# phirling/pyc2ray

Hardware: AMD Instinct MI355X
Metric: cell-updates/sec (raytrace+chem) (higher is better)
Workload: dtype f64

## Files before the change

### pyc2ray_amd/csrc/api.hip

```cpp
#include "asora_internal.hpp"

#include <chrono>

namespace asora {

static State g_state;
static std::string g_error;

State &state() { return g_state; }
int fail(int code, const std::string &msg) { g_error = msg; return code; }
void clear_error() { g_error.clear(); }

static int flush_timers()
{
    State &st = g_state;
    if (st.pending_timers.empty()) return 0;
    ASORA_HIP_TRY(hipStreamSynchronize(st.stream));
    for (hipStream_t s : st.side) if (s) ASORA_HIP_TRY(hipStreamSynchronize(s));
    for (auto &pt : st.pending_timers) {
        float ms = 0.f;
        if (hipEventElapsedTime(&ms, pt.e0, pt.e1) == hipSuccess) {
            st.k_ms[pt.which] += (double)ms;
            st.k_n[pt.which] += 1;
        }
// ... 63 lines not shown
    st.th_on = false; st.th = ThermalConsts();
    drop(st.grid[ASORA_GRID_CLUMP]);
    st.clump_mode = 0; st.clump_c = 1.0;
    st.lls_a = st.lls_b = 0.0;
    st.plane = PlaneFluxSet{};
    drop(st.budget_partial);
    if (st.budget_host) { (void)hipHostFree(st.budget_host); st.budget_host = nullptr; }
    drop(st.bubble_mask); drop(st.bubble_rows); drop(st.bubble_scan); drop(st.bubble_partial); drop(st.bubble_result); drop(st.bubble_edges);
    if (st.bubble_host) { (void)hipHostFree(st.bubble_host); st.bubble_host = nullptr; }
    drop(st.region_label); drop(st.region_volume); drop(st.region_flags); drop(st.region_result);
    drop(st.topo_complement);
    for (int g = 0; g < ASORA_GRID_COUNT; ++g) { st.grid[g] = nullptr; st.grid_valid[g] = false; }
    st.nhi = st.staging = st.acc = nullptr;
    drop(st.arena); st.arena_bytes = 0;
    st.ev_clean[0] = st.ev_clean[1] = false; st.ev_sets_known = false;
    drop(st.reach.mask); drop(st.reach.count_dev); st.reach = State::ReachMask();
    st.ev_open = false;
    st.temp_probe_valid = false;
    st.nhi_t = st.phi_t = st.heat_t = nullptr;
    st.have_heat_tables = false;
    drop(st.tables); st.table_len = 0; st.num_spec = 1; st.spec_stride = 0;
    drop(st.src_spec); drop(st.src_spec_sorted); st.src_spec_max = 0;
    drop(st.src_pos); drop(st.src_flux); drop(st.src_pos_sorted); drop(st.src_flux_sorted); st.src_i0_sorted.clear(); st.num_src = 0;
    st.src_pos_host.clear(); st.src_pos_sorted_host.clear();
    release_pair_lists(st);
    drop(st.shell_scratch); st.shell_scratch_bytes = 0;
    drop(st.sb_trail); st.sb_trail_bytes = 0;
    if (st.geom_patch_dev) { (void)hipFree(st.geom_patch_dev); st.geom_patch_dev = nullptr; st.geom_patch_cap = 0; }
    drop(st.sb_active); drop(st.sb_nbox); drop(st.sb_loss); drop(st.sb_loss_final); st.subbox_cap = 0;
    release_geometry(st);
// ... 23 lines not shown

int check_planes(const char *who, int code, const char *tail, int i_begin, int i_count)
{
    if (i_begin < 0 || i_count < 0 || i_begin + i_count > g_state.N) return fail(code, std::string(who) + ": " + tail);
    return 0;
}

int check_sources(const char *who, int code, const std::string &tail, int src_begin, int src_count)
{
    if (src_begin < 0 || src_count < 0 || src_begin + src_count > g_state.num_src) return fail(code, std::string(who) + ": " + tail);
    return 0;
}

int require_grids(const char *who, std::initializer_list<int> grids)
{
    for (int g : grids)
        if (!g_state.grid_valid[g]) return fail(4, std::string(who) + ": grid " + std::to_string(g) + " holds no data");
    return 0;
}

}

using namespace asora;

extern "C" {

constexpr int ARENA_CANDIDATES = 8;
constexpr int ARENA_SLOTS = 14;
__global__ void __launch_bounds__(256) placement_probe_kernel(char *arena, size_t slot, size_t n)
{
    const double *in[5]; double *out[7];
    for (int q = 0; q < 5; ++q) in[q] = reinterpret_cast<const double *>(arena + q * slot);
// ... 183 lines not shown
```

### pyc2ray_amd/csrc/asora_internal.hpp

```cpp
#pragma once
#include <hip/hip_runtime.h>
#include <algorithm>
#include <cmath>
#include <cstdint>
#include <cstdio>
#include <cstdlib>
#include <cstring>
#include <initializer_list>
#include <string>
#include <vector>

#include "../../include/asora_hip.h"
#include "raytrace_plan.hpp"

namespace asora {

struct OctGeomDev {
    const uint4 *cellA;
    const uint4 *cellB;
    int nsteps;
    int info;
    int inner;
    int reserved_;
};
// ... 183 lines not shown
    unsigned long long *topo_complement = nullptr;

    unsigned long long *counters = nullptr;
    long long last_gamma_cells = 0, last_eval_cells = 0;

    double *acc = nullptr;
    char *arena = nullptr;
    size_t arena_bytes = 0;
    int arena_candidates = 0;
    double arena_probe_ms = 0.0, arena_probe_worst_ms = 0.0;
    double arena_probe_wall_ms = 0.0, device_init_wall_ms = 0.0;
    int ev_base = 0;
    bool ev_clean[2] = {false, false};
    bool ev_sets_known = false;
    int ev_folded_iter = -1;
    EvolveStatus *ev_status = nullptr;
    EvolveStatus *ev_host = nullptr;
    bool ev_open = false, ev_first = true;
    double *temp_probe_dev = nullptr;
    double temp_probe[5] = {0, 0, 0, 0, 0};
    bool temp_probe_valid = false;
    double temp_consts[4] = {0, 0, 0, 0};
    int ev_reported = 0;
    int ev_enqueued = 0;
    double ev_chem[6] = {0, 0, 0, 0, 0, 0};
    int ev_src_begin = 0, ev_src_count = 0;
    RtParams ev_rt;
    bool ev_slab = false;
    int ev_own_begin = 0, ev_own_count = 0;
    bool ev_slab_passed = false;
// ... 190 lines not shown
int launch_fold_out(State &st, const double *a, const double *a_t, double *out, double *z_a, double *z_t, int i_begin, int i_count,
                    const int *done);
int launch_fold_out_pair(State &st, const double *a, const double *a_t, double *out, double *z_a, double *z_t, const double *h,
                         const double *h_t, double *hout, double *zh_a, double *zh_t, int i_begin, int i_count, const int *done);
int launch_add_planes(State &st, double *dst, const double *src, size_t n, const int *done);
int launch_convergence_test(State &st, const double *sums, EvolveStatus *status);
int launch_reach_mask(State &st, const int32_t *src_pos, int src_begin, int src_count, double R, unsigned char *mask, size_t bytes_one_layout);
int launch_reach_count(State &st, const unsigned char *mask, size_t bytes_both_layouts, unsigned long long *out_dev);

int ensure_runtime();
int require_init(const char *who);
int check_N(const char *who, int N);
int check_planes(const char *who, int code, const char *tail, int i_begin, int i_count);
int check_sources(const char *who, int code, const std::string &tail, int src_begin, int src_count);
int require_grids(const char *who, std::initializer_list<int> grids);
int ensure_optional_grid(int which);
int reset_counters();
int require_raytrace_inputs(const char *who, double R, int NumTau, bool density, bool xh_av);
void fill_rt_params(RtParams &p, double R, double sig, double dr, double minlogtau, double dlogtau, int NumTau, int radius_path = 0);
inline void use_source_list(RtParams &p, const State &st, bool sorted)
{
    p.src_pos = sorted ? st.src_pos_sorted : st.src_pos;
    p.src_flux = sorted ? st.src_flux_sorted : st.src_flux;
    p.src_spec = sorted ? st.src_spec_sorted : st.src_spec;
}
int check_source_spectra(const char *who);
void sort_sources_by_position(const int32_t *pos, int NumSrc, std::vector<int> &order);
int ensure_red_capacity(size_t entries);
int ensure_temp_probe(double bh00, double albpow, double colh0, double temph0);
ChemTileParams chem_tile_common(int i_begin, int i_count, const double chem[6]);
// ... 9 lines not shown
```

### pyc2ray_amd/csrc/bubble_mfp.hip

```cpp
#include "asora_internal.hpp"

#pragma clang fp contract(off)

namespace asora {

constexpr int BM_THREADS = 256;
constexpr int BM_WAVES = BM_THREADS / 64;
constexpr int BM_SCAN_THREADS = 1024;
constexpr int BM_SLOTS = ASORA_BUBBLE_MAX_BINS + 5;
constexpr int BM_UNDER = ASORA_BUBBLE_MAX_BINS, BM_OVER = BM_UNDER + 1, BM_ENDED = BM_UNDER + 2, BM_CAPPED = BM_UNDER + 3,
              BM_LEFT = BM_UNDER + 4;
constexpr int BM_RESULT = BM_SLOTS + 3;
constexpr int BM_BLOCKS_PER_CU = 8;
static_assert(BM_RESULT + ASORA_BUBBLE_MAX_BINS + 1 <= BUBBLE_HOST_WORDS, "the pinned area holds the result words and the edges");

__global__ void __launch_bounds__(BM_THREADS) bubble_mask_kernel(const double *__restrict__ x, int N, int W, double threshold, int phase,
                                                                 unsigned long long *__restrict__ mask, unsigned *__restrict__ rows)
{
    const int lane = threadIdx.x & 63;
    const size_t nrows = (size_t)N * N, nwaves = (size_t)gridDim.x * BM_WAVES;
    for (size_t row = (size_t)blockIdx.x * BM_WAVES + (threadIdx.x >> 6); row < nrows; row += nwaves) {
        const double *q = x + row * (size_t)N;
        unsigned long long mine = 0;
        unsigned count = 0;
// ... 225 lines not shown
        ASORA_HIP_TRY(hipGetLastError());
    }
    if (!scan) return 0;
    KernelTimer kt(ASORA_KERNEL_BUBBLE_SCAN);
    hipLaunchKernelGGL(bubble_scan_kernel, dim3(1), dim3(BM_SCAN_THREADS), 0, st.stream, (const unsigned *)st.bubble_rows, nrows,
                       st.bubble_scan);
    ASORA_HIP_TRY(hipGetLastError());
    return 0;
}

int check_bubble_grid(const char *who, int which, double threshold, int phase)
{
    const State &st = state();
    if (which < 0 || which >= ASORA_GRID_COUNT) return fail(3, std::string(who) + ": bad grid selector");
    if (!st.grid[which] || !st.grid_valid[which]) return fail(4, std::string(who) + ": grid " + std::to_string(which) + " holds no data");
    if (!std::isfinite(threshold)) return fail(3, std::string(who) + ": the threshold must be finite");
    if (phase != 0 && phase != 1) return fail(3, std::string(who) + ": phase must be 0 (x >= threshold) or 1 (x < threshold)");
    return 0;
}

struct BubbleRecord {
    int32_t *start = nullptr, *status = nullptr;
    double *dir = nullptr, *len = nullptr;
    ~BubbleRecord() { (void)hipFree(start); (void)hipFree(status); (void)hipFree(dir); (void)hipFree(len); }
};

}

using namespace asora;

// ... 96 lines not shown
```

### pyc2ray_amd/csrc/chemistry_api.hip

```cpp
#include "asora_internal.hpp"

namespace asora {

int ensure_temp_probe(double bh00, double albpow, double colh0, double temph0)
{
    State &st = state();
    const double clump = st.clump_mode == 1 ? st.clump_c : 1.0;
    const double b = clump * bh00;
    const double c[4] = {b, albpow, colh0, temph0};
    if (st.temp_probe_valid && std::memcmp(c, st.temp_consts, sizeof c) == 0 && st.temp_probe_clump == clump) return 0;
    if (!st.temp_probe_dev) ASORA_HIP_TRY(hipMalloc(&st.temp_probe_dev, sizeof(double) * 8));
    if (int rc = launch_temp_probe(st, st.grid[ASORA_GRID_TEMP], st.ncell, b, albpow, colh0, temph0, st.temp_probe_dev)) return rc;
    ASORA_HIP_TRY(hipMemcpyAsync(st.temp_probe, st.temp_probe_dev, sizeof(double) * 5, hipMemcpyDeviceToHost, st.stream));
    ASORA_HIP_TRY(hipStreamSynchronize(st.stream));
    std::memcpy(st.temp_consts, c, sizeof c);
    st.temp_probe_clump = clump;
    st.temp_probe_valid = true;
    return 0;
}

ChemTileParams chem_tile_common(int i_begin, int i_count, const double chem[6])
{
    State &st = state();
    ChemTileParams p;
// ... 35 lines not shown

using namespace asora;

extern "C" {

int asora_chemistry_device(double dt, double bh00, double albpow, double colh0, double temph0, double abu_c,
                           int *conv_flag, double *sum_xh1, double *sum_xh0)
{
    clear_error();
    if (int rc = require_init("chemistry_device")) return rc;
    State &st = state();
    if (int rc = require_grids("chemistry_device", {ASORA_GRID_NDENS, ASORA_GRID_TEMP, ASORA_GRID_XH, ASORA_GRID_XH_AV, ASORA_GRID_PHI_ION})) return rc;
    if (st.th_on) {
        if (!st.grid[ASORA_GRID_PHI_HEAT] || !st.grid_valid[ASORA_GRID_PHI_HEAT])
            return fail(4, "chemistry_device: thermal mode needs the heating rates (ASORA_GRID_PHI_HEAT) on the device");
        if (int rc = ensure_optional_grid(ASORA_GRID_TEMP_END)) return rc;
    }
    st.grid_valid[ASORA_GRID_XH_INTERMED] = true;
    ChemParams p;
    p.ncell = st.ncell;
    p.dt = dt; p.bh00 = bh00; p.albpow = albpow; p.colh0 = colh0; p.temph0 = temph0; p.abu_c = abu_c;
    p.ndens = st.grid[ASORA_GRID_NDENS]; p.temp = st.grid[ASORA_GRID_TEMP]; p.xh = st.grid[ASORA_GRID_XH];
    p.phi = st.grid[ASORA_GRID_PHI_ION];
    p.xh_av = st.grid[ASORA_GRID_XH_AV]; p.xh_intermed = st.grid[ASORA_GRID_XH_INTERMED];
    p.red_partial = st.red_partial; p.red_final = st.red_final; p.red_blocks = st.red_blocks;
    if (st.th_on) {
        p.thermal = true; p.th = st.th;
        p.phi_heat = st.grid[ASORA_GRID_PHI_HEAT]; p.temp_end = st.grid[ASORA_GRID_TEMP_END]; p.th_stats = st.th_stats_dev;
        ASORA_HIP_TRY(hipMemsetAsync(st.th_stats_dev, 0, 3 * sizeof(unsigned long long), st.stream));
        st.grid_valid[ASORA_GRID_TEMP_END] = true;
// ... 158 lines not shown
```

### pyc2ray_amd/csrc/evolve_api.hip

```cpp
#include "asora_internal.hpp"

namespace asora {

static double *acc_pair(int set) { return state().acc + (size_t)set * 2 * state().ncell; }
static double *heat_pair(int set) { return state().heat_acc + (size_t)set * 2 * state().ncell; }

static int ensure_heat_acc()
{
    State &st = state();
    if (st.heat_acc) return 0;
    ASORA_HIP_TRY(hipMalloc(&st.heat_acc, 4 * st.ncell * sizeof(double)));
    ASORA_HIP_TRY(hipMemsetAsync(st.heat_acc, 0, 4 * st.ncell * sizeof(double), st.stream));
    st.heat_clean[0] = st.heat_clean[1] = true;
    return 0;
}

static int ensure_heat_outbox()
{
    State &st = state();
    if (st.heat_outbox) return 0;
    ASORA_HIP_TRY(hipMalloc(&st.heat_outbox, st.ncell * sizeof(double)));
    return 0;
}

// ... 102 lines not shown
    if (st.th_on) {
        if (!st.have_heat_tables || st.opt[ASORA_OPT_GREY_NOTABLES])
            return fail(4, "evolve_begin: thermal mode needs heating tables on the device (heat_table_to_device)");
        if (!st.opt[ASORA_OPT_Z_TRANSPOSED]) return fail(4, "evolve_begin: thermal mode needs the [k][j][i] twins (ASORA_OPT_Z_TRANSPOSED = 1)");
        if (int rc = ensure_optional_grid(ASORA_GRID_PHI_HEAT)) return rc;
        if (int rc = ensure_optional_grid(ASORA_GRID_TEMP_END)) return rc;
        if (int rc = ensure_heat_acc()) return rc;
        if (slab) { if (int rc = ensure_heat_outbox()) return rc; }
    }
    if (int rc = check_plane_flux(st, st.plane, "evolve_begin", false, st.th_on)) return rc;
    if (slab && st.plane.count > 0 && !(own_begin == 0 && own_count == st.N))
        return fail(4, "evolve_begin_slab: a plane-parallel flux (asora_plane_flux) needs a step that owns every plane (the full-grid "
                       "exchange, asora_evolve_slab_fold_all): the slab exchange does not deliver a whole-box sweep");
    if (int rc = ensure_temp_probe(bh00, albpow, colh0, temph0)) return rc;

    if (!st.ev_sets_known || slab)
        if (int rc = zero_pairs_unless_clean()) return rc;
    if (slab) st.reach.in_use = false;
    else if (int rc = decide_reach_mask(src_begin, src_count, R, st.plane.count > 0)) return rc;

    if (!st.ev_clean[0] && !st.ev_clean[1]) return fail(11, "evolve_begin: no clean accumulator pair (internal error)");
    st.ev_base = st.ev_clean[0] ? 0 : 1;
    if (st.th_on) {
        if (int rc = zero_pairs_unless_clean(true)) return rc;
        ASORA_HIP_TRY(hipMemsetAsync(st.th_stats_dev, 0, 3 * sizeof(unsigned long long), st.stream));
    }
    st.ev_folded_iter = 0;
    if (!st.ev_status) {
        ASORA_HIP_TRY(hipMalloc(&st.ev_status, sizeof(EvolveStatus)));
        ASORA_HIP_TRY(hipHostMalloc(&st.ev_host, sizeof(EvolveStatus), hipHostMallocDefault));
// ... 97 lines not shown
    if (st.ev_slab_thermal) {
        p.heat = slab_heat_pair(0);
        st.heat_clean[0] = st.heat_clean[1] = false;
    }
    return launch_raytrace(st, p, false, st.ev_slab_thermal);
}

int asora_evolve_slab_fold_out(int i_begin, int i_count)
{
    clear_error();
    if (int rc = require_slab("evolve_slab_fold_out")) return rc;
    State &st = state();
    if (int rc = check_planes("evolve_slab_fold_out", 4, "bad plane range", i_begin, i_count)) return rc;
    if (i_count > 0 && i_begin < st.ev_own_begin + st.ev_own_count && st.ev_own_begin < i_begin + i_count)
        return fail(4, "evolve_slab_fold_out: the range holds planes this rank owns (their rates stay: the pass folds them)");
    st.ev_sets_known = false;
    double *cur = slab_pair(0), *nxt = slab_pair(1);
    if (st.ev_slab_thermal) {
        double *hcur = slab_heat_pair(0), *hnxt = slab_heat_pair(1);
        return launch_fold_out_pair(st, cur, cur + st.ncell, st.staging, nxt, nxt + st.ncell, hcur, hcur + st.ncell, st.heat_outbox,
                                    hnxt, hnxt + st.ncell, i_begin, i_count, &st.ev_status->done);
    }
    return launch_fold_out(st, cur, cur + st.ncell, st.staging, nxt, nxt + st.ncell, i_begin, i_count, &st.ev_status->done);
}

int asora_evolve_slab_fold_all(void)
{
    clear_error();
    if (int rc = require_slab("evolve_slab_fold_all")) return rc;
    State &st = state();
    if (st.ev_slab_passed) return fail(4, "evolve_slab_fold_all: the iteration's pass has been enqueued already");
    if (st.ev_own_begin != 0 || st.ev_own_count != st.N)
        return fail(4, "evolve_slab_fold_all: the step must own every plane (asora_evolve_begin_slab(..., 0, N)): the chemistry is replicated");
    st.ev_sets_known = false;
    st.ev_rates_in_outbox = true; st.ev_folded_all = true;
    double *cur = slab_pair(0), *nxt = slab_pair(1);
    if (st.ev_slab_thermal) {
        double *hcur = slab_heat_pair(0), *hnxt = slab_heat_pair(1);
        return launch_fold_out_pair(st, cur, cur + st.ncell, st.staging, nullptr, nxt + st.ncell, hcur, hcur + st.ncell, st.heat_outbox,
                                    nullptr, hnxt + st.ncell, 0, st.N, &st.ev_status->done);
    }
    return launch_fold_out(st, cur, cur + st.ncell, st.staging, nullptr, nxt + st.ncell, 0, st.N, &st.ev_status->done);
}

void *asora_evolve_slab_outbox(void) { return state().init ? (void *)state().staging : nullptr; }
void *asora_evolve_slab_heat_outbox(void) { return state().init ? (void *)state().heat_outbox : nullptr; }

static int outbox_copy(const char *who, double *box, int i_begin, int i_count, double *host, bool to_host)
// ... 77 lines not shown
}

int asora_evolve_slab_add_heat_host(int i_begin, int i_count, const double *host_planes)
{
    return slab_add_host("evolve_slab_add_heat_host", true, i_begin, i_count, host_planes);
}

int asora_evolve_slab_pass(void)
{
    clear_error();
    if (int rc = require_slab("evolve_slab_pass")) return rc;
    State &st = state();
    if (st.ev_slab_passed) return fail(4, "evolve_slab_pass: already enqueued for this iteration");
    if (st.ev_rates_in_outbox && !st.ev_folded_all)
        return fail(4, "evolve_slab_pass: this step exchanges whole grids (asora_evolve_slab_fold_all), and this iteration's fold has not been enqueued");
    st.ev_sets_known = false;
    st.ev_slab_passed = true;
    st.grid_valid[ASORA_GRID_XH_AV] = st.grid_valid[ASORA_GRID_XH_INTERMED] = true;
    st.grid_valid[ASORA_GRID_PHI_ION] = false;
    if (st.ev_slab_thermal) {
        st.heat_clean[0] = st.heat_clean[1] = false;
        st.grid_valid[ASORA_GRID_TEMP_END] = true;
        st.grid_valid[ASORA_GRID_PHI_HEAT] = false;
    }
    if (st.ev_own_count == 0) {
        ASORA_HIP_TRY(hipMemsetAsync(st.red_final, 0, sizeof(double) * 3, st.stream));
        return 0;
    }
    if (int rc = ensure_red_capacity(3 * chemistry_tile_blocks(st, st.N, st.ev_own_count))) return rc;
    ChemTileParams c = evolve_pass_params(st.ev_own_begin, st.ev_own_count, slab_set());
// ... 33 lines not shown
    st.ev_enqueued += 1;
    return 0;
}

int asora_evolve_enqueue(int iterations)
{
    clear_error();
    if (int rc = require_init("evolve_enqueue")) return rc;
    State &st = state();
    if (!st.ev_open) return fail(4, "evolve_enqueue: no evolve step in progress (call asora_evolve_begin)");
    if (st.ev_slab) return fail(4, "evolve_enqueue: the step was begun with asora_evolve_begin_slab (use the asora_evolve_slab_* calls)");
    if (iterations < 1 || iterations > EVOLVE_HIST / 2) return fail(3, "evolve_enqueue: between 1 and 32 iterations per call");
    if (st.ev_enqueued - st.ev_reported + iterations > EVOLVE_HIST)
        return fail(4, "evolve_enqueue: " + std::to_string(st.ev_enqueued - st.ev_reported) + " iterations enqueued since the last "
                           "asora_evolve_poll; the history ring holds " + std::to_string(EVOLVE_HIST) + " (poll first)");
    st.ev_sets_known = false;
    for (int it = 0; it < iterations; ++it) {
        const int set = (st.ev_base + st.ev_enqueued + it) & 1;
        if (int rc = launch_plane_flux(st, st.ev_rt, acc_pair(set), st.th_on ? heat_pair(set) : nullptr, st.th_on, &st.ev_status->done))
            return rc;
        if (st.ev_src_count > 0) {
            RtParams p = st.ev_rt;
            p.phi = acc_pair(set);
            if (st.th_on) p.heat = heat_pair(set);
            if (int rc = launch_raytrace(st, p, false, st.th_on)) return rc;
        }
        ChemTileParams c = evolve_pass_params(0, st.N, set);
        if (st.reach.in_use) { c.reach_a = st.reach.mask; c.reach_t = st.reach.mask + st.reach.bytes; }
        if (st.th_on) evolve_pass_thermal(c, set);
        if (int rc = launch_chemistry_tiles(st, c, st.stream)) return rc;
// ... 11 lines not shown
}

int asora_evolve_poll(int *niter, int *converged, double *history, int history_rows, int *rows_written)
{
    clear_error();
    if (int rc = require_init("evolve_poll")) return rc;
    State &st = state();
    if (!st.ev_open) return fail(4, "evolve_poll: no evolve step in progress (call asora_evolve_begin)");
    ASORA_HIP_TRY(hipMemcpyAsync(st.ev_host, st.ev_status, sizeof(EvolveStatus), hipMemcpyDeviceToHost, st.stream));
    ASORA_HIP_TRY(hipStreamSynchronize(st.stream));
    const EvolveStatus &h = *st.ev_host;
    const bool thermal = st.ev_slab ? st.ev_slab_thermal : st.th_on;
    if (h.niter > 0) {
        const int set = (st.ev_base + h.niter - 1) & 1;
        if (st.ev_slab && st.ev_rates_in_outbox) st.ev_folded_iter = h.niter;
        if (st.ev_folded_iter != h.niter) {
            const double *a = acc_pair(set);
            if (int rc = launch_fold_sum(st, a, a + st.ncell, st.grid[ASORA_GRID_PHI_ION])) return rc;
            if (thermal) {
                const double *hsum = heat_pair(set);
                if (int rc = launch_fold_sum(st, hsum, hsum + st.ncell, st.grid[ASORA_GRID_PHI_HEAT])) return rc;
            }
            st.ev_folded_iter = h.niter;
        }
        st.grid_valid[ASORA_GRID_PHI_ION] = true;
        st.ev_clean[set] = false; st.ev_clean[set ^ 1] = true;
        if (thermal) {
            st.grid_valid[ASORA_GRID_PHI_HEAT] = true;
            st.heat_clean[set] = false; st.heat_clean[set ^ 1] = true;
        }
    }
    st.ev_sets_known = true;
    int rows = 0;
    for (int it = st.ev_reported; it < h.niter && history && rows < history_rows; ++it, ++rows)
        for (int q = 0; q < 5; ++q) history[5 * rows + q] = h.hist[it % EVOLVE_HIST][q];
    st.ev_enqueued = h.niter;
    if (history) st.ev_reported += rows;
    else st.ev_reported = h.niter;
    if (rows_written) *rows_written = rows;
// ... 7 lines not shown
```

### pyc2ray_amd/csrc/grids_api.hip

```cpp
#include "asora_internal.hpp"
#include "rates_device.hpp"


namespace asora {

int ensure_optional_grid(int which)
{
    State &st = state();
    if ((which != ASORA_GRID_PHI_HEAT && which != ASORA_GRID_TEMP_END && which != ASORA_GRID_CLUMP) || st.grid[which]) return 0;
    const bool twin = which == ASORA_GRID_PHI_HEAT;
    ASORA_HIP_TRY(hipMalloc(&st.grid[which], (twin ? 2 : 1) * st.ncell * sizeof(double)));
    if (twin) st.heat_t = st.grid[which] + st.ncell;
    st.grid_valid[which] = false;
    return 0;
}

}

using namespace asora;

extern "C" {

int asora_grid_to_device(int which, const double *host, int N, char order)
{
    clear_error();
    if (int rc = require_init("grid_to_device")) return rc;
    if (int rc = check_N("grid_to_device", N)) return rc;
    if (which < 0 || which >= ASORA_GRID_COUNT) return fail(3, "grid_to_device: bad grid selector");
    if (!host) return fail(3, "grid_to_device: null host pointer");
    State &st = state();
    if (int rc = ensure_optional_grid(which)) return rc;
    st.zero_since_probe = std::max(st.zero_since_probe, 48);
    const size_t bytes = st.ncell * sizeof(double);
    if (order == 'C' || order == 'c') {
        ASORA_HIP_TRY(hipMemcpyAsync(st.grid[which], host, bytes, hipMemcpyHostToDevice, st.stream));
    } else if (order == 'F' || order == 'f') {
        ASORA_HIP_TRY(hipMemcpyAsync(st.staging, host, bytes, hipMemcpyHostToDevice, st.stream));
        if (int rc = launch_transpose(st, st.staging, st.grid[which], N)) return rc;
    } else
        return fail(3, "grid_to_device: order must be 'C' or 'F'");
    ASORA_HIP_TRY(hipStreamSynchronize(st.stream));
    st.grid_valid[which] = true;
    if (which == ASORA_GRID_TEMP) st.temp_probe_valid = false;
    return 0;
}

int asora_grid_to_host(int which, double *host, int N, char order)
{
    clear_error();
    if (int rc = require_init("grid_to_host")) return rc;
    if (int rc = check_N("grid_to_host", N)) return rc;
    if (which < 0 || which >= ASORA_GRID_COUNT) return fail(3, "grid_to_host: bad grid selector");
    if (!host) return fail(3, "grid_to_host: null host pointer");
    State &st = state();
    if (!st.grid[which] || !st.grid_valid[which]) return fail(3, "grid_to_host: grid " + std::to_string(which) + " holds no data");
    const size_t bytes = st.ncell * sizeof(double);
    if (order == 'C' || order == 'c') {
        ASORA_HIP_TRY(hipMemcpyAsync(host, st.grid[which], bytes, hipMemcpyDeviceToHost, st.stream));
    } else if (order == 'F' || order == 'f') {
        if (int rc = launch_transpose(st, st.grid[which], st.staging, N)) return rc;
        ASORA_HIP_TRY(hipMemcpyAsync(host, st.staging, bytes, hipMemcpyDeviceToHost, st.stream));
    } else
        return fail(3, "grid_to_host: order must be 'C' or 'F'");
    ASORA_HIP_TRY(hipStreamSynchronize(st.stream));
    return 0;
}

int asora_grid_copy(int dst, int src)
{
    clear_error();
    if (int rc = require_init("grid_copy")) return rc;
    if (dst < 0 || dst >= ASORA_GRID_COUNT || src < 0 || src >= ASORA_GRID_COUNT || dst == src)
        return fail(3, "grid_copy: bad grid selectors");
    State &st = state();
    if (!st.grid_valid[src]) return fail(3, "grid_copy: source grid holds no data");
    if (int rc = ensure_optional_grid(dst)) return rc;
    ASORA_HIP_TRY(hipMemcpyAsync(st.grid[dst], st.grid[src], st.ncell * sizeof(double), hipMemcpyDeviceToDevice,
                                 st.stream));
    st.grid_valid[dst] = true;
    if (dst == ASORA_GRID_TEMP) st.temp_probe_valid = false;
    return 0;
}

int asora_grid_scale(int which, double factor)
{
    clear_error();
    if (int rc = require_init("grid_scale")) return rc;
    if (which < 0 || which >= ASORA_GRID_COUNT) return fail(3, "grid_scale: bad grid selector");
    State &st = state();
    if (!st.grid_valid[which]) return fail(3, "grid_scale: grid " + std::to_string(which) + " holds no data");
    if (int rc = launch_scale(st, st.grid[which], st.ncell, factor)) return rc;
    if (which == ASORA_GRID_TEMP) st.temp_probe_valid = false;
    return 0;
}

int asora_grid_sum(int which, double *sum)
{
    clear_error();
    if (int rc = require_init("grid_sum")) return rc;
    if (which < 0 || which >= ASORA_GRID_COUNT) return fail(3, "grid_sum: bad grid selector");
    if (!sum) return fail(3, "grid_sum: null output pointer");
    State &st = state();
    if (!st.grid_valid[which]) return fail(3, "grid_sum: grid " + std::to_string(which) + " holds no data");
    if (!st.temp_probe_dev) ASORA_HIP_TRY(hipMalloc(&st.temp_probe_dev, sizeof(double) * 8));
    if (int rc = launch_grid_sum(st, st.grid[which], st.ncell, st.temp_probe_dev + 5)) return rc;
    ASORA_HIP_TRY(hipMemcpyAsync(sum, st.temp_probe_dev + 5, sizeof(double), hipMemcpyDeviceToHost, st.stream));
    ASORA_HIP_TRY(hipStreamSynchronize(st.stream));
    return 0;
}

int asora_host_alloc(size_t bytes, void **host)
{
    clear_error();
    if (!host || bytes == 0) return fail(3, "host_alloc: null pointer or zero size");
    *host = nullptr;
    ASORA_HIP_TRY(hipHostMalloc(host, bytes, hipHostMallocDefault));
    return 0;
}

int asora_host_free(void *host)
{
    clear_error();
    if (!host) return 0;
    ASORA_HIP_TRY(hipHostFree(host));
    return 0;
}

void *asora_device_ptr(int which)
{
    if (!state().init || which < 0 || which >= ASORA_GRID_COUNT) return nullptr;
    return state().grid[which];
}

int asora_density_to_device(const double *ndens, int N)
{
    return asora_grid_to_device(ASORA_GRID_NDENS, ndens, N, 'C');
}

static size_t rate_block_entries(int NumTau) { return std::max<size_t>(4 * (size_t)NumTau, 16); }

static int upload_rate_tables(const char *who, int NumSpec, int NumTau, const double *thin, const double *thick, const double *heat_thin,
                              const double *heat_thick)
{
    State &st = state();
    const bool heat = heat_thin && heat_thick;
// ... 201 lines not shown
        if (spec && spec_out) spec_out[s] = spec[o];
    }
    return 0;
}

int asora_planes_to_host(int which, int i_begin, int i_count, double *host)
{
    clear_error();
    if (int rc = require_init("planes_to_host")) return rc;
    State &st = state();
    if (which < 0 || which >= ASORA_GRID_COUNT) return fail(3, "planes_to_host: bad grid selector");
    if (int rc = check_planes("planes_to_host", 3, "bad plane range", i_begin, i_count)) return rc;
    if (i_count == 0) return 0;
    if (!host) return fail(3, "planes_to_host: null host pointer");
    if (!st.grid_valid[which]) return fail(3, "planes_to_host: grid " + std::to_string(which) + " holds no data");
    const size_t plane = (size_t)st.N * st.N;
    ASORA_HIP_TRY(hipMemcpyAsync(host, st.grid[which] + (size_t)i_begin * plane, (size_t)i_count * plane * sizeof(double),
                                 hipMemcpyDeviceToHost, st.stream));
    ASORA_HIP_TRY(hipStreamSynchronize(st.stream));
    return 0;
}

int asora_planes_to_device(int which, int i_begin, int i_count, const double *host)
{
    clear_error();
    if (int rc = require_init("planes_to_device")) return rc;
    State &st = state();
    if (which < 0 || which >= ASORA_GRID_COUNT) return fail(3, "planes_to_device: bad grid selector");
    if (int rc = check_planes("planes_to_device", 3, "bad plane range", i_begin, i_count)) return rc;
    if (i_count == 0) return 0;
    if (!host) return fail(3, "planes_to_device: null host pointer");
    if (int rc = ensure_optional_grid(which)) return rc;
    const size_t plane = (size_t)st.N * st.N;
    ASORA_HIP_TRY(hipMemcpyAsync(st.grid[which] + (size_t)i_begin * plane, host, (size_t)i_count * plane * sizeof(double),
                                 hipMemcpyHostToDevice, st.stream));
    ASORA_HIP_TRY(hipStreamSynchronize(st.stream));
    st.grid_valid[which] = true;
    if (which == ASORA_GRID_TEMP) st.temp_probe_valid = false;
    return 0;
}

}
```

### pyc2ray_amd/csrc/raytrace_api.hip

```cpp
#include "asora_internal.hpp"

namespace asora {

int reset_counters()
{
    State &st = state();
    ASORA_HIP_TRY(hipMemsetAsync(st.counters, 0, sizeof(unsigned long long) * COUNTER_FIELDS * COUNTER_SLOTS, st.stream));
    return 0;
}

int require_raytrace_inputs(const char *who, double R, int NumTau, bool density, bool xh_av)
{
    State &st = state();
    const std::string w = std::string(who) + ": ";
    if (int rc = check_open_boundaries(st, who, st.opt[ASORA_OPT_OPEN_BOUNDARIES] != 0, false)) return rc;
    if (density && !st.grid_valid[ASORA_GRID_NDENS]) return fail(4, w + "density not on device (density_to_device)");
    if (xh_av && !st.grid_valid[ASORA_GRID_XH_AV]) return fail(4, w + "xh_av not on device");
    if (!st.opt[ASORA_OPT_GREY_NOTABLES] && !st.tables) return fail(4, w + "radiation tables not on device (photo_table_to_device)");
    if (!(R >= 0.0)) return fail(4, w + "R must be >= 0");
    if (NumTau < 1 && !st.opt[ASORA_OPT_GREY_NOTABLES]) return fail(4, w + "NumTau must be >= 1");
    return check_source_spectra(who);
}

static int check_rt_sources(int src_begin, int src_count)
// ... 28 lines not shown
}

static int rt_begin(double R, double sig, double dr, double minlogtau, double dlogtau, int NumTau, double *dump,
                    bool pipelined = false)
{
    State &st = state();
    st.rt_open = false;
    if (int rc = require_raytrace_inputs("raytrace", R, NumTau, true, true)) return rc;

    const bool zt = st.opt[ASORA_OPT_Z_TRANSPOSED] != 0;
    const bool heat = st.opt[ASORA_OPT_HEATING] != 0 && dump == nullptr;
    if (heat && (!st.have_heat_tables || st.opt[ASORA_OPT_GREY_NOTABLES]))
        return fail(4, "raytrace: heating requested but no heating tables on device (heat_table_to_device)");
    if (int rc = check_plane_flux(st, st.plane, "raytrace", dump != nullptr, heat)) return rc;
    const size_t bytes = st.ncell * sizeof(double);
    ASORA_HIP_TRY(hipMemsetAsync(st.grid[ASORA_GRID_PHI_ION], 0, bytes, st.stream));
    if (zt) ASORA_HIP_TRY(hipMemsetAsync(st.phi_t, 0, bytes, st.stream));
    if (heat) {
        ASORA_HIP_TRY(hipMemsetAsync(st.grid[ASORA_GRID_PHI_HEAT], 0, bytes, st.stream));
        if (zt) ASORA_HIP_TRY(hipMemsetAsync(st.heat_t, 0, bytes, st.stream));
    }
    if (int rc = reset_counters()) return rc;
    if (int rc = launch_prepare_nhi(st, zt)) return rc;

    RtParams &p = st.rt_params;
    fill_rt_params(p, R, sig, dr, minlogtau, dlogtau, NumTau);
    p.dump = dump;
    if (int rc = launch_plane_flux(st, p, st.grid[ASORA_GRID_PHI_ION], st.grid[ASORA_GRID_PHI_HEAT], heat, nullptr)) return rc;
    st.rt_heat = heat;
    st.rt_pipelined = pipelined;
// ... 107 lines not shown
        sb[c] = (int)(std::lower_bound(st.src_i0_sorted.begin(), st.src_i0_sorted.end(), lo[c]) - st.src_i0_sorted.begin());
    bool reach[KMAX][KMAX];
    for (int c = 0; c < K; ++c)
        for (int d = 0; d < K; ++d) {
            bool hit = false;
            if (sb[c + 1] > sb[c])
                for (int q = lo[d]; q < lo[d + 1] && !hit; ++q) {
                    int dist = 0;
                    if (q < lo[c]) dist = std::min(lo[c] - q, q + N - (lo[c + 1] - 1));
                    else if (q >= lo[c + 1]) dist = std::min(q - (lo[c + 1] - 1), lo[c] + N - q);
                    hit = dist <= m;
                }
            reach[c][d] = hit;
        }

    ASORA_HIP_TRY(hipMemsetAsync(st.grid[ASORA_GRID_PHI_ION], 0, 2 * bytes, st.stream));
    if (int rc = reset_counters()) return rc;
    RtParams base;
    fill_rt_params(base, R, sig, dr, minlogtau, dlogtau, NumTau);
    use_source_list(base, st, true);
    base.shape_src_count = NumSrc;
    st.rt_open = false;
    ASORA_HIP_TRY(hipEventRecord(st.main_ready, st.stream));
    ASORA_HIP_TRY(hipStreamWaitEvent(up, st.main_ready, 0));
    ASORA_HIP_TRY(hipStreamWaitEvent(down, st.main_ready, 0));

    bool prepped[KMAX] = {}, traced[KMAX] = {}, sent[KMAX] = {};
    auto try_traces = [&]() -> int {
        for (int c = 0; c < K; ++c) {
            if (traced[c]) continue;
// ... 89 lines not shown
int asora_raytrace_begin_planes(double R, double sig, double dr, double minlogtau, double dlogtau, int NumTau,
                                const int *runs, int nruns)
{
    clear_error();
    if (int rc = require_init("raytrace_begin_planes")) return rc;
    State &st = state();
    st.rt_open = false;
    if (int rc = require_raytrace_inputs("raytrace_begin_planes", R, NumTau, true, true)) return rc;
    if (!st.opt[ASORA_OPT_Z_TRANSPOSED]) return fail(4, "raytrace_begin_planes: needs the [k][j][i] twins (ASORA_OPT_Z_TRANSPOSED = 1)");
    if (st.opt[ASORA_OPT_HEATING]) return fail(4, "raytrace_begin_planes: no heating rates on this path");
    if (nruns < 0 || (nruns > 0 && !runs)) return fail(3, "raytrace_begin_planes: bad plane runs");
    for (int q = 0; q < nruns; ++q)
        if (int rc = check_planes("raytrace_begin_planes", 3, "plane run outside the mesh", runs[2 * q], runs[2 * q + 1])) return rc;
    if (int rc = check_plane_flux(st, st.plane, "raytrace_begin_planes", false, false)) return rc;
    if (int rc = reset_counters()) return rc;
    if (st.plane.count > 0) {
        if (int rc = launch_prepare_range(st, 0, st.N, true, st.grid[ASORA_GRID_PHI_ION])) return rc;
    } else
        for (int q = 0; q < nruns; ++q)
            if (int rc = launch_prepare_range(st, runs[2 * q], runs[2 * q + 1], true, st.grid[ASORA_GRID_PHI_ION])) return rc;
    fill_rt_params(st.rt_params, R, sig, dr, minlogtau, dlogtau, NumTau);
    if (int rc = launch_plane_flux(st, st.rt_params, st.grid[ASORA_GRID_PHI_ION], nullptr, false, nullptr)) return rc;
    st.rt_heat = false;
    st.rt_pipelined = false;
    st.rt_by_planes = true;
    st.rt_open = true;
    return 0;
}

int asora_raytrace_range(int src_begin, int src_count)
// ... 160 lines not shown
```

### pyc2ray_amd/csrc/subbox_api.hip

```cpp
#include "asora_internal.hpp"
#include "rates_device.hpp"


namespace asora {

struct SubboxCall {
    int max_subbox, subboxsize;
    float loss_fraction;
    double sig, dr, R, minlogtau, dlogtau;
    int NumTau, table_len;
    const double2 *tables;
    const int32_t *src_pos;
    const int32_t *host_pos;
    const double *src_flux;
    int src_begin, src_count;
    bool heat, keep_heat;
    double *dump;
};

static int refuse_source_spectra(const char *who)
{
    if (!state().src_spec) return 0;
    return fail(4, std::string(who) + ": the sub-box raytracer has one spectrum for all sources, and the sources on the device "
                                      "carry table sets of their own (source_spectra_to_device); use raytrace_device / evolve3D");
}

static int subbox_core(const SubboxCall &c, long long &total_nbox, double &total_loss)
{
    State &st = state();
    const int N = st.N;
    const size_t bytes = st.ncell * sizeof(double);
    const bool grey = st.opt[ASORA_OPT_GREY_NOTABLES] != 0;
    ASORA_HIP_TRY(hipMemsetAsync(st.grid[ASORA_GRID_PHI_ION], 0, 2 * bytes, st.stream));
    if (c.heat) {
        if (!c.keep_heat) ASORA_HIP_TRY(hipMemsetAsync(st.grid[ASORA_GRID_PHI_HEAT], 0, bytes, st.stream));
        ASORA_HIP_TRY(hipMemsetAsync(st.heat_t, 0, bytes, st.stream));
    }
    if (c.dump) ASORA_HIP_TRY(hipMemsetAsync(c.dump, 0, bytes, st.stream));
    if (int rc = launch_prepare_nhi(st, true)) return rc;
    if (int rc = ensure_logtab(st)) return rc;

    const int ext_r = std::min(c.max_subbox, N / 2 - 1 + N % 2);
    const int ext_l = std::min(c.max_subbox, N / 2);
    const int S_all = std::max(ext_r, ext_l);
    const bool range_open = ext_r > 0 && ext_l > 0;

    SubboxParams p;
// ... 283 lines not shown
```

Measured before the change: 116.5 billion.

## Defer the evolve poll's rate fold until a consumer needs the grid

The evolve poll no longer folds the accumulated ionization/heating rate pairs into the PHI grids eagerly. It records a pending fold and settles it lazily: completed when a reader (grid_to_host, grid_sum, chemistry, device_ptr, etc.) touches the grid, or cancelled when the grid is about to be overwritten (new raytrace, evolve_enqueue, host upload). This avoids a fold kernel per poll when the rates are discarded. The risk is a missed settle point that would leave a consumer reading stale rates.

Result: no change. 117.5 billion (median of 6 runs) (+0.9%).

```diff
diff --git a/pyc2ray_amd/csrc/api.hip b/pyc2ray_amd/csrc/api.hip
--- a/pyc2ray_amd/csrc/api.hip
+++ b/pyc2ray_amd/csrc/api.hip
@@ -101,6 +101,7 @@
     st.nhi = st.staging = st.acc = nullptr;
     drop(st.arena); st.arena_bytes = 0;
     st.ev_clean[0] = st.ev_clean[1] = false; st.ev_sets_known = false;
+    (void)settle_pending_fold(FOLD_CANCEL);
     drop(st.reach.mask); drop(st.reach.count_dev); st.reach = State::ReachMask();
     st.ev_open = false;
     st.temp_probe_valid = false;
@@ -154,8 +155,10 @@
 
 int require_grids(const char *who, std::initializer_list<int> grids)
 {
-    for (int g : grids)
+    for (int g : grids) {
         if (!g_state.grid_valid[g]) return fail(4, std::string(who) + ": grid " + std::to_string(g) + " holds no data");
+        if (int rc = settle_pending_fold(FOLD_COMPLETE, fold_grid_bit(g))) return rc;
+    }
     return 0;
 }
 
diff --git a/pyc2ray_amd/csrc/asora_internal.hpp b/pyc2ray_amd/csrc/asora_internal.hpp
--- a/pyc2ray_amd/csrc/asora_internal.hpp
+++ b/pyc2ray_amd/csrc/asora_internal.hpp
@@ -221,6 +221,7 @@
     bool ev_clean[2] = {false, false};
     bool ev_sets_known = false;
     int ev_folded_iter = -1;
+    struct PendingFold { bool ion = false, heat = false; int set = 0, iter = 0; } ev_pending;
     EvolveStatus *ev_status = nullptr;
     EvolveStatus *ev_host = nullptr;
     bool ev_open = false, ev_first = true;
@@ -441,6 +442,14 @@
 int check_planes(const char *who, int code, const char *tail, int i_begin, int i_count);
 int check_sources(const char *who, int code, const std::string &tail, int src_begin, int src_count);
 int require_grids(const char *who, std::initializer_list<int> grids);
+enum FoldSettle {
+    FOLD_NOTHING_PENDING = 0,
+    FOLD_COMPLETE,
+    FOLD_CANCEL
+};
+constexpr unsigned FOLD_ION = 1u, FOLD_HEAT = 2u, FOLD_BOTH = 3u;
+inline unsigned fold_grid_bit(int which) { return which == ASORA_GRID_PHI_ION ? FOLD_ION : which == ASORA_GRID_PHI_HEAT ? FOLD_HEAT : 0u; }
+int settle_pending_fold(FoldSettle how, unsigned grids = FOLD_BOTH);
 int ensure_optional_grid(int which);
 int reset_counters();
 int require_raytrace_inputs(const char *who, double R, int NumTau, bool density, bool xh_av);
diff --git a/pyc2ray_amd/csrc/bubble_mfp.hip b/pyc2ray_amd/csrc/bubble_mfp.hip
--- a/pyc2ray_amd/csrc/bubble_mfp.hip
+++ b/pyc2ray_amd/csrc/bubble_mfp.hip
@@ -263,6 +263,7 @@
     const State &st = state();
     if (which < 0 || which >= ASORA_GRID_COUNT) return fail(3, std::string(who) + ": bad grid selector");
     if (!st.grid[which] || !st.grid_valid[which]) return fail(4, std::string(who) + ": grid " + std::to_string(which) + " holds no data");
+    if (int rc = settle_pending_fold(FOLD_COMPLETE, fold_grid_bit(which))) return rc;
     if (!std::isfinite(threshold)) return fail(3, std::string(who) + ": the threshold must be finite");
     if (phase != 0 && phase != 1) return fail(3, std::string(who) + ": phase must be 0 (x >= threshold) or 1 (x < threshold)");
     return 0;
diff --git a/pyc2ray_amd/csrc/chemistry_api.hip b/pyc2ray_amd/csrc/chemistry_api.hip
--- a/pyc2ray_amd/csrc/chemistry_api.hip
+++ b/pyc2ray_amd/csrc/chemistry_api.hip
@@ -73,6 +73,7 @@
     if (st.th_on) {
         if (!st.grid[ASORA_GRID_PHI_HEAT] || !st.grid_valid[ASORA_GRID_PHI_HEAT])
             return fail(4, "chemistry_device: thermal mode needs the heating rates (ASORA_GRID_PHI_HEAT) on the device");
+        if (int rc = settle_pending_fold(FOLD_COMPLETE, FOLD_HEAT)) return rc;
         if (int rc = ensure_optional_grid(ASORA_GRID_TEMP_END)) return rc;
     }
     st.grid_valid[ASORA_GRID_XH_INTERMED] = true;
diff --git a/pyc2ray_amd/csrc/evolve_api.hip b/pyc2ray_amd/csrc/evolve_api.hip
--- a/pyc2ray_amd/csrc/evolve_api.hip
+++ b/pyc2ray_amd/csrc/evolve_api.hip
@@ -4,6 +4,28 @@
 
 static double *acc_pair(int set) { return state().acc + (size_t)set * 2 * state().ncell; }
 static double *heat_pair(int set) { return state().heat_acc + (size_t)set * 2 * state().ncell; }
+
+int settle_pending_fold(FoldSettle how, unsigned grids)
+{
+    State &st = state();
+    State::PendingFold &pf = st.ev_pending;
+    const bool ion = pf.ion && (grids & FOLD_ION), heat = pf.heat && (grids & FOLD_HEAT);
+    if (how == FOLD_NOTHING_PENDING || !(ion || heat)) return 0;
+    if (how == FOLD_COMPLETE) {
+        if (ion) {
+            const double *a = acc_pair(pf.set);
+            if (int rc = launch_fold_sum(st, a, a + st.ncell, st.grid[ASORA_GRID_PHI_ION])) return rc;
+        }
+        if (heat) {
+            const double *hsum = heat_pair(pf.set);
+            if (int rc = launch_fold_sum(st, hsum, hsum + st.ncell, st.grid[ASORA_GRID_PHI_HEAT])) return rc;
+        }
+    }
+    if (ion) pf.ion = false;
+    if (heat) pf.heat = false;
+    if (!pf.ion && !pf.heat) st.ev_folded_iter = pf.iter;
+    return 0;
+}
 
 static int ensure_heat_acc()
 {
@@ -140,6 +162,7 @@
                        "exchange, asora_evolve_slab_fold_all): the slab exchange does not deliver a whole-box sweep");
     if (int rc = ensure_temp_probe(bh00, albpow, colh0, temph0)) return rc;
 
+    if (int rc = settle_pending_fold(FOLD_COMPLETE)) return rc;
     if (!st.ev_sets_known || slab)
         if (int rc = zero_pairs_unless_clean()) return rc;
     if (slab) st.reach.in_use = false;
@@ -267,6 +290,7 @@
     if (int rc = check_planes("evolve_slab_fold_out", 4, "bad plane range", i_begin, i_count)) return rc;
     if (i_count > 0 && i_begin < st.ev_own_begin + st.ev_own_count && st.ev_own_begin < i_begin + i_count)
         return fail(4, "evolve_slab_fold_out: the range holds planes this rank owns (their rates stay: the pass folds them)");
+    if (i_count > 0) { if (int rc = settle_pending_fold(FOLD_COMPLETE)) return rc; }
     st.ev_sets_known = false;
     double *cur = slab_pair(0), *nxt = slab_pair(1);
     if (st.ev_slab_thermal) {
@@ -285,6 +309,7 @@
     if (st.ev_slab_passed) return fail(4, "evolve_slab_fold_all: the iteration's pass has been enqueued already");
     if (st.ev_own_begin != 0 || st.ev_own_count != st.N)
         return fail(4, "evolve_slab_fold_all: the step must own every plane (asora_evolve_begin_slab(..., 0, N)): the chemistry is replicated");
+    if (int rc = settle_pending_fold(FOLD_COMPLETE)) return rc;
     st.ev_sets_known = false;
     st.ev_rates_in_outbox = true; st.ev_folded_all = true;
     double *cur = slab_pair(0), *nxt = slab_pair(1);
@@ -392,6 +417,7 @@
     if (st.ev_slab_passed) return fail(4, "evolve_slab_pass: already enqueued for this iteration");
     if (st.ev_rates_in_outbox && !st.ev_folded_all)
         return fail(4, "evolve_slab_pass: this step exchanges whole grids (asora_evolve_slab_fold_all), and this iteration's fold has not been enqueued");
+    (void)settle_pending_fold(FOLD_CANCEL);
     st.ev_sets_known = false;
     st.ev_slab_passed = true;
     st.grid_valid[ASORA_GRID_XH_AV] = st.grid_valid[ASORA_GRID_XH_INTERMED] = true;
@@ -455,6 +481,8 @@
     if (st.ev_enqueued - st.ev_reported + iterations > EVOLVE_HIST)
         return fail(4, "evolve_enqueue: " + std::to_string(st.ev_enqueued - st.ev_reported) + " iterations enqueued since the last "
                            "asora_evolve_poll; the history ring holds " + std::to_string(EVOLVE_HIST) + " (poll first)");
+    (void)settle_pending_fold(FOLD_CANCEL, FOLD_ION);
+    if (int rc = settle_pending_fold(st.th_on ? FOLD_CANCEL : FOLD_COMPLETE, FOLD_HEAT)) return rc;
     st.ev_sets_known = false;
     for (int it = 0; it < iterations; ++it) {
         const int set = (st.ev_base + st.ev_enqueued + it) & 1;
@@ -496,15 +524,12 @@
     if (h.niter > 0) {
         const int set = (st.ev_base + h.niter - 1) & 1;
         if (st.ev_slab && st.ev_rates_in_outbox) st.ev_folded_iter = h.niter;
-        if (st.ev_folded_iter != h.niter) {
-            const double *a = acc_pair(set);
-            if (int rc = launch_fold_sum(st, a, a + st.ncell, st.grid[ASORA_GRID_PHI_ION])) return rc;
-            if (thermal) {
-                const double *hsum = heat_pair(set);
-                if (int rc = launch_fold_sum(st, hsum, hsum + st.ncell, st.grid[ASORA_GRID_PHI_HEAT])) return rc;
-            }
-            st.ev_folded_iter = h.niter;
+        const bool owed = (st.ev_pending.ion || st.ev_pending.heat) && st.ev_pending.iter == h.niter;
+        if (st.ev_folded_iter != h.niter && !owed) {
+            st.ev_pending.ion = true; st.ev_pending.heat = thermal;
+            st.ev_pending.set = set; st.ev_pending.iter = h.niter;
         }
+        if (h.done) { if (int rc = settle_pending_fold(FOLD_COMPLETE)) return rc; }
         st.grid_valid[ASORA_GRID_PHI_ION] = true;
         st.ev_clean[set] = false; st.ev_clean[set ^ 1] = true;
         if (thermal) {
diff --git a/pyc2ray_amd/csrc/grids_api.hip b/pyc2ray_amd/csrc/grids_api.hip
--- a/pyc2ray_amd/csrc/grids_api.hip
+++ b/pyc2ray_amd/csrc/grids_api.hip
@@ -32,6 +32,8 @@
     if (int rc = ensure_optional_grid(which)) return rc;
     st.zero_since_probe = std::max(st.zero_since_probe, 48);
     const size_t bytes = st.ncell * sizeof(double);
+    if (order == 'C' || order == 'c' || order == 'F' || order == 'f')
+        (void)settle_pending_fold(FOLD_CANCEL, fold_grid_bit(which));
     if (order == 'C' || order == 'c') {
         ASORA_HIP_TRY(hipMemcpyAsync(st.grid[which], host, bytes, hipMemcpyHostToDevice, st.stream));
     } else if (order == 'F' || order == 'f') {
@@ -54,6 +56,7 @@
     if (!host) return fail(3, "grid_to_host: null host pointer");
     State &st = state();
     if (!st.grid[which] || !st.grid_valid[which]) return fail(3, "grid_to_host: grid " + std::to_string(which) + " holds no data");
+    if (int rc = settle_pending_fold(FOLD_COMPLETE, fold_grid_bit(which))) return rc;
     const size_t bytes = st.ncell * sizeof(double);
     if (order == 'C' || order == 'c') {
         ASORA_HIP_TRY(hipMemcpyAsync(host, st.grid[which], bytes, hipMemcpyDeviceToHost, st.stream));
@@ -74,7 +77,9 @@
         return fail(3, "grid_copy: bad grid selectors");
     State &st = state();
     if (!st.grid_valid[src]) return fail(3, "grid_copy: source grid holds no data");
+    if (int rc = settle_pending_fold(FOLD_COMPLETE, fold_grid_bit(src))) return rc;
     if (int rc = ensure_optional_grid(dst)) return rc;
+    (void)settle_pending_fold(FOLD_CANCEL, fold_grid_bit(dst));
     ASORA_HIP_TRY(hipMemcpyAsync(st.grid[dst], st.grid[src], st.ncell * sizeof(double), hipMemcpyDeviceToDevice,
                                  st.stream));
     st.grid_valid[dst] = true;
@@ -89,6 +94,7 @@
     if (which < 0 || which >= ASORA_GRID_COUNT) return fail(3, "grid_scale: bad grid selector");
     State &st = state();
     if (!st.grid_valid[which]) return fail(3, "grid_scale: grid " + std::to_string(which) + " holds no data");
+    if (int rc = settle_pending_fold(FOLD_COMPLETE, fold_grid_bit(which))) return rc;
     if (int rc = launch_scale(st, st.grid[which], st.ncell, factor)) return rc;
     if (which == ASORA_GRID_TEMP) st.temp_probe_valid = false;
     return 0;
@@ -102,6 +108,7 @@
     if (!sum) return fail(3, "grid_sum: null output pointer");
     State &st = state();
     if (!st.grid_valid[which]) return fail(3, "grid_sum: grid " + std::to_string(which) + " holds no data");
+    if (int rc = settle_pending_fold(FOLD_COMPLETE, fold_grid_bit(which))) return rc;
     if (!st.temp_probe_dev) ASORA_HIP_TRY(hipMalloc(&st.temp_probe_dev, sizeof(double) * 8));
     if (int rc = launch_grid_sum(st, st.grid[which], st.ncell, st.temp_probe_dev + 5)) return rc;
     ASORA_HIP_TRY(hipMemcpyAsync(sum, st.temp_probe_dev + 5, sizeof(double), hipMemcpyDeviceToHost, st.stream));
@@ -129,6 +136,7 @@
 void *asora_device_ptr(int which)
 {
     if (!state().init || which < 0 || which >= ASORA_GRID_COUNT) return nullptr;
+    if (settle_pending_fold(FOLD_COMPLETE, fold_grid_bit(which))) return nullptr;
     return state().grid[which];
 }
 
@@ -360,6 +368,7 @@
     if (i_count == 0) return 0;
     if (!host) return fail(3, "planes_to_host: null host pointer");
     if (!st.grid_valid[which]) return fail(3, "planes_to_host: grid " + std::to_string(which) + " holds no data");
+    if (int rc = settle_pending_fold(FOLD_COMPLETE, fold_grid_bit(which))) return rc;
     const size_t plane = (size_t)st.N * st.N;
     ASORA_HIP_TRY(hipMemcpyAsync(host, st.grid[which] + (size_t)i_begin * plane, (size_t)i_count * plane * sizeof(double),
                                  hipMemcpyDeviceToHost, st.stream));
@@ -377,6 +386,7 @@
     if (i_count == 0) return 0;
     if (!host) return fail(3, "planes_to_device: null host pointer");
     if (int rc = ensure_optional_grid(which)) return rc;
+    if (int rc = settle_pending_fold(i_count == st.N ? FOLD_CANCEL : FOLD_COMPLETE, fold_grid_bit(which))) return rc;
     const size_t plane = (size_t)st.N * st.N;
     ASORA_HIP_TRY(hipMemcpyAsync(st.grid[which] + (size_t)i_begin * plane, host, (size_t)i_count * plane * sizeof(double),
                                  hipMemcpyHostToDevice, st.stream));
diff --git a/pyc2ray_amd/csrc/raytrace_api.hip b/pyc2ray_amd/csrc/raytrace_api.hip
--- a/pyc2ray_amd/csrc/raytrace_api.hip
+++ b/pyc2ray_amd/csrc/raytrace_api.hip
@@ -66,6 +66,7 @@
         return fail(4, "raytrace: heating requested but no heating tables on device (heat_table_to_device)");
     if (int rc = check_plane_flux(st, st.plane, "raytrace", dump != nullptr, heat)) return rc;
     const size_t bytes = st.ncell * sizeof(double);
+    (void)settle_pending_fold(FOLD_CANCEL, heat ? FOLD_BOTH : FOLD_ION);
     ASORA_HIP_TRY(hipMemsetAsync(st.grid[ASORA_GRID_PHI_ION], 0, bytes, st.stream));
     if (zt) ASORA_HIP_TRY(hipMemsetAsync(st.phi_t, 0, bytes, st.stream));
     if (heat) {
@@ -203,6 +204,7 @@
             reach[c][d] = hit;
         }
 
+    (void)settle_pending_fold(FOLD_CANCEL, FOLD_ION);
     ASORA_HIP_TRY(hipMemsetAsync(st.grid[ASORA_GRID_PHI_ION], 0, 2 * bytes, st.stream));
     if (int rc = reset_counters()) return rc;
     RtParams base;
@@ -322,6 +324,7 @@
         if (int rc = check_planes("raytrace_begin_planes", 3, "plane run outside the mesh", runs[2 * q], runs[2 * q + 1])) return rc;
     if (int rc = check_plane_flux(st, st.plane, "raytrace_begin_planes", false, false)) return rc;
     if (int rc = reset_counters()) return rc;
+    if (int rc = settle_pending_fold(FOLD_COMPLETE, FOLD_ION)) return rc;
     if (st.plane.count > 0) {
         if (int rc = launch_prepare_range(st, 0, st.N, true, st.grid[ASORA_GRID_PHI_ION])) return rc;
     } else
diff --git a/pyc2ray_amd/csrc/subbox_api.hip b/pyc2ray_amd/csrc/subbox_api.hip
--- a/pyc2ray_amd/csrc/subbox_api.hip
+++ b/pyc2ray_amd/csrc/subbox_api.hip
@@ -31,6 +31,8 @@
     const int N = st.N;
     const size_t bytes = st.ncell * sizeof(double);
     const bool grey = st.opt[ASORA_OPT_GREY_NOTABLES] != 0;
+    (void)settle_pending_fold(FOLD_CANCEL, FOLD_ION);
+    if (c.heat) { if (int rc = settle_pending_fold(c.keep_heat ? FOLD_COMPLETE : FOLD_CANCEL, FOLD_HEAT)) return rc; }
     ASORA_HIP_TRY(hipMemsetAsync(st.grid[ASORA_GRID_PHI_ION], 0, 2 * bytes, st.stream));
     if (c.heat) {
         if (!c.keep_heat) ASORA_HIP_TRY(hipMemsetAsync(st.grid[ASORA_GRID_PHI_HEAT], 0, bytes, st.stream));
```
